# wkentaro/chainer-mask-rcnn

Measured on AMD Instinct MI355X. Metric: images/sec train step, ResNet50-C4 Mask R-CNN, COCO 800x1333, higher is better.
Workload: dtype f32 (bf16x3 split operands, f32 accumulate)

## Files before the change

chainer_mask_rcnn_amd/csrc/conv_gemm.hip:

```cpp
#include <algorithm>
#include <cstring>
#include <type_traits>

#include "common.h"

namespace {

typedef float f32x16 __attribute__((ext_vector_type(16)));

constexpr int BK = 32;
constexpr bool single_buffered(int tm, int mode)
{
    if (tm == 1) return mode == 0;
    return tm >= 2 && (mode == 0 || mode == 2);
}
constexpr int min_blocks(int tm, int mode)
{
    if (!single_buffered(tm, mode)) return 1;
    return tm == 4 ? 2 : (tm == 2 ? 3 : 6);
}
constexpr int KPAD = 4;

enum Mode { FWD = 0, DGRAD = 1, WGRAD = 2 };
constexpr bool is_fwd(int m) { return m == FWD; }
// ... 972 lines not shown
                    }
                }
                float row_scale[EG];
                if (MODE == WGRAD && p.scale) {
#pragma unroll
                    for (int q = 0; q < EG; ++q) {
                        const int e = g * EG + q;
                        const int row = m0 + wm * (32 * TM) + i * 32 + (e & 3) + 8 * (e >> 2) + 4 * lk;
                        row_scale[q] = row < p.M ? p.scale[row] : 0.f;
                    }
                }
#pragma unroll
                for (int q = 0; q < EG; ++q) {
                    float v = acc[i][j][g * EG + q];
                    if (MODE != WGRAD) {
                        if (f_bias) v += bias;
                        if (f_aff) v = v * scale + shift;
                        if (f_res) v += aux0[q];
                        if (f_acc) v += aux1[q];
                        if (f_resy) v += aux2[q] > 0.f ? aux0[q] : 0.f;
                        else if (f_resg) v += aux0[q];
                        if (f_relu) v = fmaxf(v, 0.f);
                        if (f_outm) v = aux3[q] > 0.f ? v : 0.f;
                    } else if (p.scale) {
                        v *= row_scale[q];
                    }
                    bstore1(rC, off[q], v);
                }
            }
        }
    }
}

__global__ void splitk_reduce_kernel(const float *__restrict__ ws, int splits, int64_t n,
                                     int64_t stride, float *__restrict__ out)
{
    const int64_t nv = n / 4;
    for (int64_t i = (int64_t)blockIdx.x * blockDim.x + threadIdx.x; i < nv;
         i += (int64_t)gridDim.x * blockDim.x) {
        float4 a = reinterpret_cast<const float4 *>(ws)[i];
        int s = 1;
        for (; s + 4 <= splits; s += 4) {
            const float4 v0 = reinterpret_cast<const float4 *>(ws + (s + 0) * stride)[i];
            const float4 v1 = reinterpret_cast<const float4 *>(ws + (s + 1) * stride)[i];
            const float4 v2 = reinterpret_cast<const float4 *>(ws + (s + 2) * stride)[i];
            const float4 v3 = reinterpret_cast<const float4 *>(ws + (s + 3) * stride)[i];
            a.x += v0.x; a.y += v0.y; a.z += v0.z; a.w += v0.w;
            a.x += v1.x; a.y += v1.y; a.z += v1.z; a.w += v1.w;
            a.x += v2.x; a.y += v2.y; a.z += v2.z; a.w += v2.w;
            a.x += v3.x; a.y += v3.y; a.z += v3.z; a.w += v3.w;
        }
        for (; s < splits; ++s) {
            const float4 v = reinterpret_cast<const float4 *>(ws + s * stride)[i];
            a.x += v.x; a.y += v.y; a.z += v.z; a.w += v.w;
        }
        reinterpret_cast<float4 *>(out)[i] = a;
    }
}

constexpr int64_t kSlotsBig = 512, kSlotsSmall = 1024;

int g_split_bf16 = 3;
int g_big_split_k = -1;
int g_big_split_min_slices = 16;
int g_w8_min_k = 256;
int g_w8 = 1;

int g_pw = 3;

inline bool pw_plain(const GemmParams &p)
{
    return p.R == 1 && p.S == 1 && p.stride == 1 && p.pad == 0 && p.perm_n == 0 && !p.stem && p.gp == p.sh &&
           p.gq == p.sw && p.out_mode == OUT_PLAIN;
}

inline bool k3_plain(const GemmParams &p)
{
    return p.R == 3 && p.S == 3 && p.stride == 1 && p.pad == 1 && p.perm_n == 0 && !p.stem &&
           p.out_mode == OUT_PLAIN;
}

template <int TM, int TN, int MODE>
void launch_kernel(const GemmParams &p, int64_t tiles, int splits, hipStream_t s, int batch = 1)
{
    hipEvent_t ev0, ev1;
    mrcnn::prof_take(&ev0, &ev1);
    auto go = [&](auto kernel) {
        hipExtLaunchKernelGGL(kernel, dim3((unsigned)tiles, splits, batch), dim3(256), 0, s, ev0, ev1, 0, p);
// ... 50 lines not shown
                        : (MODE == FWD ? mrcnn::PROF_CONV_FWD_128 : mrcnn::PROF_CONV_DGRAD_128) + (TM >= 2 ? 0 : 1);
    return mrcnn::ProfKernelScope(kind, flops, bytes);
}

template <int TM, int TN, int MODE>
void launch_tiles(GemmParams p, int m_lo, int m_hi, int splits, hipStream_t s)
{
    constexpr int BM = 64 * TM, BN = 64 * TN;
    p.m_lo = m_lo;
    p.M = m_hi;
    const int64_t blocks = mrcnn::ceil_div(m_hi - m_lo, BM) * mrcnn::ceil_div(p.N, BN);
    if (blocks <= 0) return;
    const auto prof = gemm_prof<TM, MODE>(p, m_hi - m_lo);
    launch_kernel<TM, TN, MODE>(p, blocks, splits, s);
}

constexpr int64_t kSplitWsBytes = 192ll << 20;

struct FixParams {
    const float *ws;
    float *C;
    const float *bias, *scale, *shift, *residual, *res_g, *res_y, *out_mask_y;
    int splits, rows, N, row0, ldc, flags;
    int perm_n, pq;
    int64_t stride;
};

__global__ void __launch_bounds__(256) splitk_epilogue_kernel(const FixParams f)
{
    const int n4 = f.N / 4;
    const int64_t i = (int64_t)blockIdx.x * blockDim.x + threadIdx.x;
    if (i >= (int64_t)f.rows * n4) return;
    const int r = (int)(i / n4), c = (int)(i - (int64_t)r * n4) * 4;
    float4 a = *reinterpret_cast<const float4 *>(f.ws + (int64_t)r * f.N + c);
    for (int s = 1; s < f.splits; ++s) {
        const float4 v = *reinterpret_cast<const float4 *>(f.ws + s * f.stride + (int64_t)r * f.N + c);
        a.x += v.x; a.y += v.y; a.z += v.z; a.w += v.w;
    }
    float v[4] = {a.x, a.y, a.z, a.w};
    int orow = f.row0 + r;
    if (f.perm_n > 0) {
        const PermRow pr = perm_row(orow, f.pq);
        if (pr.n >= f.perm_n) return;
        orow = pr.n * f.pq + pr.pos;
    }
    const int64_t off = (int64_t)orow * f.ldc + c;
#pragma unroll
    for (int k = 0; k < 4; ++k) {
        float x = v[k];
        if (f.flags & MRCNN_EPI_BIAS) x += f.bias[c + k];
        if (f.flags & MRCNN_EPI_AFFINE) x = x * f.scale[c + k] + (f.shift ? f.shift[c + k] : 0.f);
        if (f.flags & MRCNN_EPI_RESIDUAL) x += f.residual[off + k];
        if (f.flags & MRCNN_EPI_ACCUM) x += f.C[off + k];
        if (f.res_g) x += (!f.res_y || f.res_y[off + k] > 0.f) ? f.res_g[off + k] : 0.f;
        if (f.flags & MRCNN_EPI_RELU) x = fmaxf(x, 0.f);
        if (f.out_mask_y) x = f.out_mask_y[off + k] > 0.f ? x : 0.f;
        v[k] = x;
    }
    *reinterpret_cast<float4 *>(f.C + off) = make_float4(v[0], v[1], v[2], v[3]);
}

template <int MODE>
bool can_split_rows(const GemmParams &p)
{
    return p.split_ws && MODE != WGRAD && p.out_mode == OUT_PLAIN && !p.stem && p.N % 4 == 0 &&
           p.ldc == p.N;
}

int64_t fit_ws(int64_t splits, int64_t rows, int N)
{
    while (splits > 1 && rows * N * splits * 4 > kSplitWsBytes) --splits;
    return splits;
}

int64_t k_splits(int total_slices, int depth_div, int64_t target_wgs, int64_t tiles, int64_t rows, int N,
                 int64_t cap)
{
    return fit_ws(std::min<int64_t>(std::min<int64_t>(cap, total_slices / depth_div),
                                    mrcnn::ceil_div(target_wgs, tiles)),
                  rows, N);
}

template <int MODE>
void slab_sum(const GemmParams &p, int rows_lo, int splits, hipStream_t s)
{
    const int rows = p.M - rows_lo;
    FixParams f = {};
    f.ws = p.split_ws; f.C = p.C;
    f.bias = p.bias; f.scale = p.scale; f.shift = p.shift; f.residual = p.residual;
// ... 567 lines not shown
    p.scale = out_row_scale;
    p.M = Kout; p.N = R * S * C; p.Kc = (int)pixels;
    p.gp = P; p.gq = Q; p.sh = H; p.sw = W;
    p.R = R; p.S = S; p.stride = stride; p.pad = pad;
    p.lda = C; p.ldg = ldg; p.cin = C; p.ldc = R * S * C;
    const int64_t gwsz = (int64_t)Kout * R * S * C;
    const int64_t big = mrcnn::ceil_div(p.M, 128) * mrcnn::ceil_div(p.N, 128);
    const int64_t small = mrcnn::ceil_div(p.M, 64) * mrcnn::ceil_div(p.N, 64);
    const int64_t max_splits = std::min<int64_t>(64, std::max<int64_t>(1, pixels / (8 * BK)));
    const bool use_big = p.N > 64 && p.M > 64 && (big * max_splits * 2 >= kSlotsBig || g_big_min_tiles <= 1);
    const int64_t tiles = use_big ? big : small;
    if (C % (use_big ? 128 : 64) == 0 && N_ >= BK)
        p.perm_n = choose_perm(N_, P, Q, R, S, stride, pad);
    const int64_t k_extent = p.perm_n ? mrcnn::ceil_div(N_, BK) * BK * P * Q : pixels;
    const bool split_kernel = (g_split_bf16 & 1) && p.perm_n == 0;
    const int64_t slots_big = !split_kernel && single_buffered(2, WGRAD) ? 768 : kSlotsBig;
    int splits = wgrad_splits(tiles, pixels, use_big ? slots_big : kSlotsSmall);
    if (!ws) splits = 1;
    p.split_len = (int)(mrcnn::ceil_div(mrcnn::ceil_div(k_extent, splits), BK) * BK);
    splits = (int)mrcnn::ceil_div(k_extent, p.split_len);
    p.split_stride = gwsz;
    if (int rc = set_extents(p, pixels * ldg, (int64_t)N_ * H * W * C, gwsz)) return rc;
    p.C = splits > 1 ? (float *)ws : gw;
    {
        mrcnn::ProfKernelScope prof(use_big ? mrcnn::PROF_CONV_WGRAD_128 : mrcnn::PROF_CONV_WGRAD_64,
                                    2.0 * p.M * p.N * (double)pixels,
                                    4.0 * ((double)p.M * p.N + (double)pixels * (p.M + (double)C)));
        if (use_big)
            launch_kernel<2, 2, WGRAD>(p, big, splits, s);
        else
            launch_kernel<1, 1, WGRAD>(p, tiles, splits, s);
    }
    if (splits > 1) {
        const int64_t blocks = mrcnn::ceil_div(gwsz / 4, 256);
        hipLaunchKernelGGL(splitk_reduce_kernel, dim3((unsigned)blocks), dim3(256), 0, s,
                           (const float *)ws, splits, gwsz, gwsz, gw);
    }
    return mrcnn::check_launch("conv_wgrad");
}

extern "C" int mrcnn_conv2d_wgrad_ex(const mrcnn_conv_desc *d, const float *x, const float *gy,
                                     float *gw, void *ws, const float *out_row_scale,
                                     void *stream)
{
    if (int rc = check_desc(d)) return rc;
    MRCNN_REQUIRE(x && gy && gw, "conv2d_wgrad: null pointer");
    MRCNN_REQUIRE(aligned16(x) && aligned16(gy) && aligned16(gw) && (!ws || aligned16(ws)),
                  "conv2d_wgrad: pointers must be 16-byte aligned");
    return wgrad_impl(gy, d->K, x, gw, d->K, (int64_t)d->N * d->P * d->Q, d->N, d->H, d->W, d->C,
                      d->P, d->Q, d->R, d->S, d->stride, d->pad, ws, mrcnn::as_stream(stream),
                      out_row_scale);
}

extern "C" int mrcnn_conv2d_wgrad(const mrcnn_conv_desc *d, const float *x, const float *gy,
                                  float *gw, void *ws, void *stream)
{
    return mrcnn_conv2d_wgrad_ex(d, x, gy, gw, ws, nullptr, stream);
}

extern "C" int mrcnn_deconv2x2s2_fwd(const float *x, const float *w, const float *bias, float *y,
                                     int N, int H, int W, int C, int K, int epi_flags,
                                     void *stream)
{
    MRCNN_REQUIRE(x && w && y, "deconv_fwd: null pointer");
    MRCNN_REQUIRE(N > 0 && H > 0 && W > 0 && C > 0 && K > 0 && C % 4 == 0 && K % 4 == 0,
                  "deconv_fwd: bad shape");
    MRCNN_REQUIRE(aligned16(x) && aligned16(w), "deconv_fwd: x/w must be 16-byte aligned");
    MRCNN_REQUIRE((epi_flags & ~(MRCNN_EPI_BIAS | MRCNN_EPI_RELU)) == 0, "deconv_fwd: bad flags");
// ... 59 lines not shown
```

chainer_mask_rcnn_amd/csrc/conv_winograd.h:

```cpp
#pragma once

namespace {

constexpr int kXi = 36;

struct F2 { float x, y; };
__device__ __forceinline__ F2 operator+(F2 a, F2 b) { return {a.x + b.x, a.y + b.y}; }
__device__ __forceinline__ F2 operator-(F2 a, F2 b) { return {a.x - b.x, a.y - b.y}; }
__device__ __forceinline__ F2 operator*(float s, F2 a) { return {s * a.x, s * a.y}; }

template <typename T>
__device__ __forceinline__ void wino_bt(const T (&d)[6], T (&t)[6])
{
    t[0] = d[0] - 1.5f * d[1] - 2.f * d[2] + 1.5f * d[3] + d[4];
    t[1] = 2.5f * d[3] + 0.5f * d[2] - d[1] + d[4];
    t[2] = d[1] - 2.5f * d[2] + 0.5f * d[3] + d[4];
    t[3] = 2.f * (d[3] - d[1]) - d[2] + d[4];
    t[4] = 0.5f * (d[1] - d[3]) - d[2] + d[4];
    t[5] = d[1] - 1.5f * d[2] - 2.f * d[3] + 1.5f * d[4] + d[5];
}
template <typename T>
__device__ __forceinline__ void wino_at(const T (&m)[6], T (&y)[4])
{
    const T s12 = m[1] + m[2], d12 = m[1] - m[2];
// ... 79 lines not shown
#pragma unroll
        for (int i = 0; i < D; ++i) col[i] = d[i][j];
        if constexpr (GRAD_TILE) wino_g4(col, o);
        else wino_bt(col, o);
#pragma unroll
        for (int a = 0; a < 6; ++a) t[a][j] = o[a];
    }
    float *out = v + tile * C + c;
    const int64_t xi_stride = T * C;
#pragma unroll
    for (int a = 0; a < 6; ++a) {
        F2 o[6];
        if constexpr (GRAD_TILE) wino_g4(t[a], o);
        else wino_bt(t[a], o);
#pragma unroll
        for (int b = 0; b < 6; ++b)
            *reinterpret_cast<F2 *>(out + (a * 6 + b) * xi_stride) = o[b];
    }
}

struct WinoOutParams {
    const float *m;
    float *y;
    const float *scale, *shift, *mask;
    int H, W, K, TH, TW, flags;
    int64_t T;
    int *fix_count;
    int2 *fix_list;
    int fix_cap;
    float ambiguity;
};
float g_wino_ambiguity = 4e-6f;

template <bool FIXUP>
__global__ void __launch_bounds__(256) wino_output_transform_kernel(const WinoOutParams p)
{
    const int k2n = p.K >> 1;
    const int64_t idx = (int64_t)blockIdx.x * 256 + threadIdx.x;
    if (idx >= p.T * k2n) return;
    const int64_t tile = idx / k2n;
    const int k = (int)(idx - tile * k2n) * 2;
    const int tx = (int)(tile % p.TW);
    const int64_t q = tile / p.TW;
    const int ty = (int)(q % p.TH);
    const int64_t n = q / p.TH;
    const float *in = p.m + tile * p.K + k;
    const int64_t xi_stride = p.T * p.K;
    F2 m[6][6];
#pragma unroll
    for (int a = 0; a < 6; ++a)
#pragma unroll
        for (int b = 0; b < 6; ++b)
            m[a][b] = *reinterpret_cast<const F2 *>(in + (a * 6 + b) * xi_stride);
    const int y0 = 4 * ty, x0 = 4 * tx;
    const int64_t obase = (n * p.H * p.W) * p.K + k;
    F2 mk[4][4];
    if (p.mask) {
#pragma unroll
        for (int i = 0; i < 4; ++i)
#pragma unroll
            for (int j = 0; j < 4; ++j) {
                const bool ok = y0 + i < p.H && x0 + j < p.W;
                mk[i][j] = ok ? *reinterpret_cast<const F2 *>(
                                    p.mask + obase + ((int64_t)(y0 + i) * p.W + x0 + j) * p.K)
                              : F2{0.f, 0.f};
            }
    }
    F2 s[4][6];
    F2 sa[FIXUP ? 4 : 1][6];
#pragma unroll
    for (int b = 0; b < 6; ++b) {
        F2 col[6], o[4];
#pragma unroll
        for (int a = 0; a < 6; ++a) col[a] = m[a][b];
        wino_at(col, o);
#pragma unroll
        for (int i = 0; i < 4; ++i) s[i][b] = o[i];
        if constexpr (FIXUP) {
#pragma unroll
            for (int a = 0; a < 6; ++a) col[a] = F2{fabsf(col[a].x), fabsf(col[a].y)};
            wino_at_abs(col, o);
#pragma unroll
            for (int i = 0; i < 4; ++i) sa[i][b] = o[i];
        }
    }
    F2 sc = {1.f, 1.f}, sh = {0.f, 0.f};
    const bool aff = (p.flags & (MRCNN_EPI_AFFINE | MRCNN_EPI_BIAS)) != 0;
    const bool relu = (p.flags & MRCNN_EPI_RELU) != 0;
    if (aff) {
        if (p.scale) sc = *reinterpret_cast<const F2 *>(p.scale + k);
        if (p.shift) sh = *reinterpret_cast<const F2 *>(p.shift + k);
    }
#pragma unroll
    for (int i = 0; i < 4; ++i) {
        F2 o[4], ob[4];
        wino_at(s[i], o);
        if constexpr (FIXUP) wino_at_abs(sa[i], ob);
#pragma unroll
        for (int j = 0; j < 4; ++j) {
            if (y0 + i >= p.H || x0 + j >= p.W) continue;
            F2 v = o[j];
            if (aff) { v.x = v.x * sc.x + sh.x; v.y = v.y * sc.y + sh.y; }
            if constexpr (FIXUP) {
                const float bx = p.ambiguity * ob[j].x * fabsf(sc.x);
                const float by = p.ambiguity * ob[j].y * fabsf(sc.y);
                const int pix = (int)(n * p.H * p.W) + (y0 + i) * p.W + x0 + j;
                if (fabsf(v.x) < bx) {
                    const int at = atomicAdd(p.fix_count, 1);
                    if (at < p.fix_cap) p.fix_list[at] = make_int2(pix, k);
                }
                if (fabsf(v.y) < by) {
                    const int at = atomicAdd(p.fix_count, 1);
                    if (at < p.fix_cap) p.fix_list[at] = make_int2(pix, k + 1);
                }
            }
            if (relu) { v.x = fmaxf(v.x, 0.f); v.y = fmaxf(v.y, 0.f); }
            if (p.mask) {
                v.x = mk[i][j].x > 0.f ? v.x : 0.f;
                v.y = mk[i][j].y > 0.f ? v.y : 0.f;
            }
            *reinterpret_cast<F2 *>(p.y + obase + ((int64_t)(y0 + i) * p.W + x0 + j) * p.K) = v;
        }
    }
}

struct WinoFixParams {
    const float *x, *w, *scale, *shift;
    float *y;
    const int *count;
    const int2 *list;
    int cap, H, W, C, K, flags;
};
__global__ void __launch_bounds__(256) wino_fixup_kernel(const WinoFixParams p)
{
    const int lane = threadIdx.x & 63;
    const int wave = (int)((blockIdx.x * 256 + threadIdx.x) >> 6), nwaves = (int)(gridDim.x * 4);
    const int n_items = min(*p.count, p.cap);
    for (int it = wave; it < n_items; it += nwaves) {
        const int2 e = p.list[it];
        const int pix = e.x, k = e.y;
        const int n = pix / (p.H * p.W), rem = pix - n * (p.H * p.W);
        const int yy = rem / p.W, xx = rem - yy * p.W;
        float acc = 0.f;
        for (int r = 0; r < 3; ++r) {
            const int iy = yy + r - 1;
            if ((unsigned)iy >= (unsigned)p.H) continue;
            for (int s = 0; s < 3; ++s) {
                const int ix = xx + s - 1;
                if ((unsigned)ix >= (unsigned)p.W) continue;
                const float *xp = p.x + ((int64_t)(n * p.H + iy) * p.W + ix) * p.C;
                const float *wp = p.w + ((int64_t)k * 9 + r * 3 + s) * p.C;
                for (int c = lane * 4; c < p.C; c += 256) {
                    const float4 a = *reinterpret_cast<const float4 *>(xp + c);
                    const float4 b = *reinterpret_cast<const float4 *>(wp + c);
                    acc += (a.x * b.x + a.y * b.y) + (a.z * b.z + a.w * b.w);
                }
            }
        }
#pragma unroll
        for (int off = 32; off > 0; off >>= 1) acc += __shfl_down(acc, off, 64);
        if (lane == 0) {
            float v = acc;
            if (p.flags & (MRCNN_EPI_AFFINE | MRCNN_EPI_BIAS))
                v = v * (p.scale ? p.scale[k] : 1.f) + (p.shift ? p.shift[k] : 0.f);
            if (p.flags & MRCNN_EPI_RELU) v = fmaxf(v, 0.f);
            p.y[(int64_t)pix * p.K + k] = v;
        }
    }
}

template <bool TRANSPOSED>
__global__ void __launch_bounds__(256) wino_filter_transform_kernel(
    const float *__restrict__ w, float *__restrict__ u, int K, int C,
    const float *__restrict__ row_scale)
{
    __shared__ float tile[32][33];
    const int k0 = blockIdx.y * 32, c0 = blockIdx.x * 32;
    const int tx = threadIdx.x & 31, ty = threadIdx.x >> 5;
    double f[4][9];
#pragma unroll
    for (int j = 0; j < 4; ++j) {
        const int k = k0 + ty + 8 * j, c = c0 + tx;
        const bool ok = k < K && c < C;
        const double rsc = (TRANSPOSED && row_scale && ok) ? (double)row_scale[k] : 1.0;
#pragma unroll
        for (int rs = 0; rs < 9; ++rs) {
            const int src = TRANSPOSED ? 8 - rs : rs;
            f[j][rs] = ok ? (double)w[((int64_t)k * 9 + src) * C + c] * rsc : 0.0;
        }
    }
    for (int a = 0; a < 6; ++a)
        for (int b = 0; b < 6; ++b) {
            float val[4];
#pragma unroll
            for (int j = 0; j < 4; ++j) {
                double acc = 0.0;
#pragma unroll
                for (int r = 0; r < 3; ++r) {
                    const double row = kFilterG[b][0] * f[j][r * 3] + kFilterG[b][1] * f[j][r * 3 + 1] +
                                       kFilterG[b][2] * f[j][r * 3 + 2];
                    acc += kFilterG[a][r] * row;
                }
                val[j] = (float)acc;
            }
            float *dst = u + (int64_t)(a * 6 + b) * K * C;
            if constexpr (!TRANSPOSED) {
#pragma unroll
                for (int j = 0; j < 4; ++j) {
                    const int k = k0 + ty + 8 * j, c = c0 + tx;
                    if (k < K && c < C) dst[(int64_t)k * C + c] = val[j];
                }
            } else {
                __syncthreads();
#pragma unroll
                for (int j = 0; j < 4; ++j) tile[ty + 8 * j][tx] = val[j];
                __syncthreads();
#pragma unroll
                for (int j = 0; j < 4; ++j) {
                    const int c = c0 + ty + 8 * j, k = k0 + tx;
                    if (c < C && k < K) dst[(int64_t)c * K + k] = tile[tx][ty + 8 * j];
                }
            }
        }
}

__global__ void __launch_bounds__(256) wino_wgrad_finish_kernel(
    const float *__restrict__ slabs, int splits, int64_t split_stride, float *__restrict__ gw,
    const float *__restrict__ row_scale, int K, int C)
{
    const int64_t idx = (int64_t)blockIdx.x * 256 + threadIdx.x;
    if (idx >= (int64_t)K * C) return;
    const int k = (int)(idx / C), c = (int)(idx - (int64_t)k * C);
    const int64_t kc = (int64_t)K * C;
    float du[kXi];
#pragma unroll
    for (int xi = 0; xi < kXi; ++xi) du[xi] = slabs[xi * kc + idx];
    for (int s = 1; s < splits; ++s) {
        const float *sl = slabs + s * split_stride;
#pragma unroll
        for (int xi = 0; xi < kXi; ++xi) du[xi] += sl[xi * kc + idx];
    }
    const double rsc = row_scale ? (double)row_scale[k] : 1.0;
    double t[3][6];
#pragma unroll
    for (int r = 0; r < 3; ++r)
#pragma unroll
        for (int b = 0; b < 6; ++b) {
            double acc = 0.0;
#pragma unroll
            for (int a = 0; a < 6; ++a) acc += kWgradAT[r][a] * (double)du[a * 6 + b];
            t[r][b] = acc;
        }
#pragma unroll
    for (int r = 0; r < 3; ++r)
#pragma unroll
        for (int s = 0; s < 3; ++s) {
// ... 68 lines not shown
        launch_kernel<1, 1, FWD>(q, mrcnn::ceil_div(p.N, 64), 1, s, kXi);
    } else if (big) {
        launch_kernel<2, 2, FWD>(p, tiles, 1, s, kXi);
    } else {
        launch_kernel<1, 1, FWD>(p, tiles, 1, s, kXi);
    }
    return mrcnn::check_launch("wino_batched_gemm");
}

}

extern "C" int64_t mrcnn_conv3x3_wino_v_bytes(const mrcnn_conv_desc *d)
{
    return d ? 4 * wino_plane_floats(d, d->C) : 0;
}

extern "C" int64_t mrcnn_conv3x3_wino_workspace_bytes(const mrcnn_conv_desc *d)
{
    if (!d) return 0;
    const int64_t ch = std::max(d->C, d->K);
    return 4 * ((1 + kWinoMaxSplits) * wino_u_floats(d) + 2 * wino_plane_floats(d, (int)ch));
}

extern "C" int64_t mrcnn_conv3x3_wino_u_bytes(const mrcnn_conv_desc *d)
{
    return d ? 4 * wino_u_floats(d) : 0;
}

extern "C" int mrcnn_conv3x3_wino_filter(const mrcnn_conv_desc *d, const float *w, float *u,
                                         void *stream)
{
    if (int rc = wino_check(d, "conv3x3_wino_filter")) return rc;
    MRCNN_REQUIRE(w && u, "conv3x3_wino_filter: null pointer");
    hipLaunchKernelGGL((wino_filter_transform_kernel<false>),
                       dim3((d->C + 31) / 32, (d->K + 31) / 32), dim3(256), 0,
                       mrcnn::as_stream(stream), w, u, d->K, d->C, (const float *)nullptr);
    return mrcnn::check_launch("conv3x3_wino_filter");
}

extern "C" int mrcnn_conv3x3_wino_fwd(const mrcnn_conv_desc *d, const float *x, const float *w,
                                      const float *u_pre, const float *scale, const float *shift,
                                      float *y, int epi_flags, float *v, void *ws, void *stream)
{
    if (int rc = wino_check(d, "conv3x3_wino_fwd")) return rc;
    MRCNN_REQUIRE(x && (w || u_pre) && y && ws, "conv3x3_wino_fwd: null pointer");
    MRCNN_REQUIRE((epi_flags & ~(MRCNN_EPI_AFFINE | MRCNN_EPI_BIAS | MRCNN_EPI_RELU |
                                 MRCNN_EPI_EXACT_SIGNS)) == 0,
                  "conv3x3_wino_fwd: only AFFINE or BIAS, RELU and EXACT_SIGNS");
    MRCNN_REQUIRE(!(epi_flags & MRCNN_EPI_EXACT_SIGNS) || w,
                  "conv3x3_wino_fwd: EXACT_SIGNS needs the filter itself");
    MRCNN_REQUIRE(!(epi_flags & MRCNN_EPI_AFFINE) || scale, "conv3x3_wino_fwd: affine flag without scale");
    MRCNN_REQUIRE(!(epi_flags & MRCNN_EPI_BIAS) || (shift && !scale && !(epi_flags & MRCNN_EPI_AFFINE)),
                  "conv3x3_wino_fwd: the bias flag takes the bias in `shift` and excludes AFFINE");
    hipStream_t s = mrcnn::as_stream(stream);
    const WinoGeom g = wino_geom(d);
    float *u_ws = (float *)ws;
    float *m = u_ws + wino_u_floats(d);
    float *vbuf = v ? v : m + wino_plane_floats(d, d->K);
    const float *u = u_pre;
    if (!u) {
        hipLaunchKernelGGL((wino_filter_transform_kernel<false>),
                           dim3((d->C + 31) / 32, (d->K + 31) / 32), dim3(256), 0, s, w, u_ws, d->K,
                           d->C, (const float *)nullptr);
        u = u_ws;
    }
    wino_launch_data_transform<false>(x, vbuf, g, d->C, s);
    if (int rc = wino_batched_gemm(vbuf, u, m, g.T, d->K, d->C, s)) return rc;
    WinoOutParams o = {};
    o.m = m; o.y = y; o.scale = scale; o.shift = shift;
    o.H = d->H; o.W = d->W; o.K = d->K; o.TH = g.TH; o.TW = g.TW;
    o.flags = epi_flags & ~MRCNN_EPI_EXACT_SIGNS; o.T = g.T;
    const bool fixup = (epi_flags & MRCNN_EPI_EXACT_SIGNS) != 0;
    if (fixup) {
        float *fix = (float *)ws + wino_u_floats(d) + 2 * wino_plane_floats(d, std::max(d->C, d->K));
        o.fix_count = (int *)fix;
        o.fix_list = (int2 *)(fix + 4);
        o.fix_cap = (int)std::min<int64_t>(1 << 20, (8 * wino_u_floats(d) - 4) / 2);
        o.ambiguity = g_wino_ambiguity;
        MRCNN_HIP_TRY(hipMemsetAsync(o.fix_count, 0, 16, s));
    }
    {
        mrcnn::ProfScope prof(mrcnn::PROF_WINO_TRANSFORM, 0.,
                              4.0 * d->K * (36.0 * g.T + (double)d->N * d->H * d->W), s);
        const dim3 grid((unsigned)mrcnn::ceil_div(g.T * (d->K / 2), 256));
        if (fixup) hipLaunchKernelGGL(wino_output_transform_kernel<true>, grid, dim3(256), 0, s, o);
        else hipLaunchKernelGGL(wino_output_transform_kernel<false>, grid, dim3(256), 0, s, o);
    }
    if (fixup) {
        WinoFixParams f = {};
        f.x = x; f.w = w; f.scale = scale; f.shift = shift; f.y = y;
        f.count = o.fix_count; f.list = o.fix_list; f.cap = o.fix_cap;
        f.H = d->H; f.W = d->W; f.C = d->C; f.K = d->K; f.flags = o.flags;
        hipLaunchKernelGGL(wino_fixup_kernel, dim3(1024), dim3(256), 0, s, f);
    }
    return mrcnn::check_launch("conv3x3_wino_fwd");
}

extern "C" int mrcnn_conv3x3_wino_dgrad(const mrcnn_conv_desc *d, const float *gy, const float *w,
                                        const float *w_row_scale, float *gx,
                                        const float *out_scale, const float *out_mask_y, void *ws,
                                        void *stream)
{
    if (int rc = wino_check(d, "conv3x3_wino_dgrad")) return rc;
    MRCNN_REQUIRE(gy && w && gx && ws, "conv3x3_wino_dgrad: null pointer");
    hipStream_t s = mrcnn::as_stream(stream);
    const WinoGeom g = wino_geom(d);
    const int64_t ch = std::max(d->C, d->K);
    float *u = (float *)ws;
    float *gt = u + (1 + kWinoMaxSplits) * wino_u_floats(d);
    float *m = gt + wino_plane_floats(d, (int)ch);
    hipLaunchKernelGGL((wino_filter_transform_kernel<true>),
                       dim3((d->C + 31) / 32, (d->K + 31) / 32), dim3(256), 0, s, w, u, d->K, d->C,
                       w_row_scale);
    wino_launch_data_transform<false>(gy, gt, g, d->K, s);
    if (int rc = wino_batched_gemm(gt, u, m, g.T, d->C, d->K, s)) return rc;
    WinoOutParams o = {};
    o.m = m; o.y = gx; o.scale = out_scale; o.mask = out_mask_y;
    o.H = d->H; o.W = d->W; o.K = d->C; o.TH = g.TH; o.TW = g.TW;
    o.flags = out_scale ? MRCNN_EPI_AFFINE : 0; o.T = g.T;
    {
        mrcnn::ProfScope prof(mrcnn::PROF_WINO_TRANSFORM, 0.,
                              4.0 * d->C * (36.0 * g.T + (out_mask_y ? 2.0 : 1.0) * d->N * d->H * d->W), s);
        hipLaunchKernelGGL(wino_output_transform_kernel<false>,
                           dim3((unsigned)mrcnn::ceil_div(g.T * (d->C / 2), 256)), dim3(256), 0, s, o);
    }
    return mrcnn::check_launch("conv3x3_wino_dgrad");
}

extern "C" int mrcnn_conv3x3_wino_wgrad(const mrcnn_conv_desc *d, const float *x, const float *v,
                                        const float *gy, float *gw, const float *out_row_scale,
                                        void *ws, void *stream)
{
    if (int rc = wino_check(d, "conv3x3_wino_wgrad")) return rc;
    MRCNN_REQUIRE((x != nullptr) != (v != nullptr), "conv3x3_wino_wgrad: exactly one of x / v");
    MRCNN_REQUIRE(gy && gw && ws, "conv3x3_wino_wgrad: null pointer");
    hipStream_t s = mrcnn::as_stream(stream);
    const WinoGeom g = wino_geom(d);
    float *slabs = (float *)ws + wino_u_floats(d);
    float *gt = (float *)ws + (1 + kWinoMaxSplits) * wino_u_floats(d);
    if (!v) {
        float *vx = gt + wino_plane_floats(d, std::max(d->C, d->K));
        wino_launch_data_transform<false>(x, vx, g, d->C, s);
        v = vx;
    }
    wino_launch_data_transform<true>(gy, gt, g, d->K, s);
    GemmParams p = {};
    p.A = gt; p.B = v;
    p.M = d->K; p.N = d->C; p.Kc = (int)g.T;
    p.gp = p.gq = p.sh = p.sw = 1;
    p.R = p.S = 1; p.stride = 1; p.pad = 0;
    p.lda = d->C; p.ldg = d->K; p.cin = d->C; p.ldc = d->C;
    const int64_t kc = (int64_t)d->K * d->C;
    const bool big = p.M > 64 && p.N > 64;
    const int64_t tiles = big ? mrcnn::ceil_div(p.M, 128) * mrcnn::ceil_div(p.N, 128)
                              : mrcnn::ceil_div(p.M, 64) * mrcnn::ceil_div(p.N, 64);
    const int64_t slots = big ? (single_buffered(2, WGRAD) ? 768 : kSlotsBig) : kSlotsSmall;
    int splits = std::min(kWinoMaxSplits, wgrad_splits(tiles * kXi, g.T, slots));
// ... 30 lines not shown
```

chainer_mask_rcnn_amd/csrc/elementwise.hip:

```cpp
#include <algorithm>

#include "common.h"

namespace {

constexpr int kColsumSplits = 128;

__global__ void affine_fwd_kernel(const float *__restrict__ x, const float *__restrict__ W,
                                  const float *__restrict__ b, float *__restrict__ y,
                                  int64_t total, int C)
{
    for (int64_t i = (int64_t)blockIdx.x * blockDim.x + threadIdx.x; i < total;
         i += (int64_t)gridDim.x * blockDim.x) {
        const int c = (int)(i % C);
        y[i] = W[c] * x[i] + b[c];
    }
}

template <bool VEC>
__global__ void epilogue_bwd_kernel(const float *__restrict__ gy, const float *__restrict__ y,
                                    const float *__restrict__ scale, float *__restrict__ g,
                                    int64_t total, int C)
{
    if (VEC) {
// ... 67 lines not shown
        for (; s < splits; s += 4) a0 += partial[(int64_t)s * C + c];
    }
    red[g][cx] = (a0 + a1) + (a2 + a3);
    __syncthreads();
    if (g == 0 && c < C) out[c] = (red[0][cx] + red[1][cx]) + (red[2][cx] + red[3][cx]);
}

template <typename V>
__device__ __forceinline__ V vmax(V a, V b);
template <> __device__ __forceinline__ float vmax(float a, float b) { return fmaxf(a, b); }
template <> __device__ __forceinline__ float4 vmax(float4 a, float4 b)
{
    return make_float4(fmaxf(a.x, b.x), fmaxf(a.y, b.y), fmaxf(a.z, b.z), fmaxf(a.w, b.w));
}
template <typename V> __device__ __forceinline__ V vneginf();
template <> __device__ __forceinline__ float vneginf() { return -INFINITY; }
template <> __device__ __forceinline__ float4 vneginf()
{
    return make_float4(-INFINITY, -INFINITY, -INFINITY, -INFINITY);
}

template <typename V>
__global__ void maxpool_kernel(const V *__restrict__ x, V *__restrict__ y, int N, int H, int W,
                               int CV, int P, int Q)
{
    const int64_t total = (int64_t)N * P * Q * CV;
    for (int64_t i = (int64_t)blockIdx.x * blockDim.x + threadIdx.x; i < total;
         i += (int64_t)gridDim.x * blockDim.x) {
        const int c = (int)(i % CV);
        int64_t t = i / CV;
        const int q = (int)(t % Q); t /= Q;
        const int p = (int)(t % P);
        const int n = (int)(t / P);
        V m = vneginf<V>();
#pragma unroll
        for (int r = 0; r < 3; ++r) {
            const int iy = 2 * p - 1 + r;
            if (iy < 0 || iy >= H) continue;
#pragma unroll
            for (int s = 0; s < 3; ++s) {
                const int ix = 2 * q - 1 + s;
                if (ix < 0 || ix >= W) continue;
                m = vmax(m, x[(((int64_t)n * H + iy) * W + ix) * CV + c]);
            }
        }
        y[i] = m;
    }
}

template <bool VEC>
__global__ void avgpool_fwd_kernel(const float *__restrict__ x, float *__restrict__ y, int R,
                                   int HW, int C)
{
    const int w = VEC ? 4 : 1;
    const int cv = C / w;
    const int64_t i = (int64_t)blockIdx.x * blockDim.x + threadIdx.x;
    if (i >= (int64_t)R * cv) return;
    const int r = (int)(i / cv), c = (int)(i % cv);
    const float inv = 1.f / (float)HW;
    if (VEC) {
        const float4 *p = reinterpret_cast<const float4 *>(x) + (int64_t)r * HW * cv + c;
        float4 a = make_float4(0.f, 0.f, 0.f, 0.f);
        for (int k = 0; k < HW; ++k) {
            const float4 v = p[(int64_t)k * cv];
            a.x += v.x; a.y += v.y; a.z += v.z; a.w += v.w;
        }
        reinterpret_cast<float4 *>(y)[i] = make_float4(a.x * inv, a.y * inv, a.z * inv, a.w * inv);
    } else {
        const float *p = x + (int64_t)r * HW * C + c;
        float a = 0.f;
        for (int k = 0; k < HW; ++k) a += p[(int64_t)k * C];
        y[i] = a * inv;
    }
}

template <bool VEC>
__global__ void avgpool_bwd_kernel(const float *__restrict__ gy, float *__restrict__ gx, int R,
// ... 232 lines not shown
namespace {
__global__ void __launch_bounds__(256)
sparse3x3_gather_kernel(const float4 *__restrict__ x, const float4 *__restrict__ g,
                        const int32_t *__restrict__ rows, int H, int W, int C4, int K4,
                        float4 *__restrict__ patches, float4 *__restrict__ g_rows)
{
    const int i = blockIdx.x, t = blockIdx.y;
    const int p = rows[i];
    if (t == 9) {
        const float4 *src = g + (int64_t)p * K4;
        float4 *dst = g_rows + (int64_t)i * K4;
        for (int c = threadIdx.x; c < K4; c += blockDim.x) dst[c] = src[c];
        return;
    }
    const int px = p % W, py = (p / W) % H, n = p / (W * H);
    const int yy = py + t / 3 - 1, xx = px + t % 3 - 1;
    const bool in = (unsigned)yy < (unsigned)H && (unsigned)xx < (unsigned)W;
    const float4 *src = x + (((int64_t)n * H + yy) * W + xx) * C4;
    float4 *dst = patches + ((int64_t)i * 9 + t) * C4;
    const float4 zero = make_float4(0.f, 0.f, 0.f, 0.f);
    for (int c = threadIdx.x; c < C4; c += blockDim.x) dst[c] = in ? src[c] : zero;
}

__global__ void __launch_bounds__(256)
sparse3x3_scatter_kernel(const float4 *__restrict__ gp, const int32_t *__restrict__ lookup, int H,
                         int W, int C4, float4 *__restrict__ gx)
{
    const int q = blockIdx.x;
    const int qx = q % W, qy = (q / W) % H, n = q / (W * H);
    int src[9];
#pragma unroll
    for (int t = 0; t < 9; ++t) {
        const int yy = qy - (t / 3 - 1), xx = qx - (t % 3 - 1);
        src[t] = ((unsigned)yy < (unsigned)H && (unsigned)xx < (unsigned)W)
                     ? lookup[((int64_t)n * H + yy) * W + xx] : -1;
    }
    for (int c = threadIdx.x; c < C4; c += blockDim.x) {
        float4 acc = make_float4(0.f, 0.f, 0.f, 0.f);
#pragma unroll
        for (int t = 0; t < 9; ++t) {
            if (src[t] < 0) continue;
            const float4 v = gp[((int64_t)src[t] * 9 + t) * C4 + c];
            acc.x += v.x; acc.y += v.y; acc.z += v.z; acc.w += v.w;
        }
        gx[(int64_t)q * C4 + c] = acc;
    }
}
}

extern "C" int mrcnn_sparse3x3_gather(const float *x, const float *g, const int32_t *rows,
                                      int n_rows, int N, int H, int W, int C, int K,
                                      float *patches, float *g_rows, void *stream)
{
    MRCNN_REQUIRE(n_rows >= 0 && N > 0 && H > 0 && W > 0 && C > 0 && K > 0 && C % 4 == 0 &&
                      K % 4 == 0, "sparse3x3_gather: bad shape");
    if (n_rows == 0) return 0;
    MRCNN_REQUIRE(x && g && rows && patches && g_rows, "sparse3x3_gather: null pointer");
    mrcnn::ProfScope prof(mrcnn::PROF_ELEMENTWISE, 0.,
                          8.0 * (double)n_rows * (9.0 * C + K), mrcnn::as_stream(stream));
    hipLaunchKernelGGL(sparse3x3_gather_kernel, dim3(n_rows, 10), dim3(256), 0,
                       mrcnn::as_stream(stream), (const float4 *)x, (const float4 *)g, rows, H, W,
                       C / 4, K / 4, (float4 *)patches, (float4 *)g_rows);
    return mrcnn::check_launch("sparse3x3_gather");
}

extern "C" int mrcnn_sparse3x3_scatter(const float *g_patches, const int32_t *lookup, int N, int H,
                                       int W, int C, float *gx, void *stream)
{
    MRCNN_REQUIRE(N > 0 && H > 0 && W > 0 && C > 0 && C % 4 == 0, "sparse3x3_scatter: bad shape");
    MRCNN_REQUIRE((int64_t)N * H * W < (int64_t)INT32_MAX, "sparse3x3_scatter: map too large");
    MRCNN_REQUIRE(g_patches && lookup && gx, "sparse3x3_scatter: null pointer");
    hipLaunchKernelGGL(sparse3x3_scatter_kernel, dim3(N * H * W), dim3(256), 0,
                       mrcnn::as_stream(stream), (const float4 *)g_patches, lookup, H, W, C / 4,
                       (float4 *)gx);
    return mrcnn::check_launch("sparse3x3_scatter");
}

extern "C" int mrcnn_sgd_momentum_wd_ex(float *p, float *g, float *v, int64_t n, float lr,
// ... 25 lines not shown
```

Before: 90.92.

## Batch loads ahead of use in reduce, epilogue, winograd, pooling and scatter kernels

Several memory-bound helper kernels are restructured so that their global loads are issued unconditionally up front, using clamped or dummy addresses, before any data-dependent branching. This raises memory-level parallelism in the split-K reduce and epilogue, the winograd output and filter transforms, max pooling and the sparse 3x3 scatter. The winograd filter transform gets a new thread mapping with an LDS transpose tile, the masked output transform becomes a template specialisation, and the reduce launch uses smaller blocks for small outputs. The cost is some extra loads and more register pressure.

```diff
diff --git a/chainer_mask_rcnn_amd/csrc/conv_gemm.hip b/chainer_mask_rcnn_amd/csrc/conv_gemm.hip
--- a/chainer_mask_rcnn_amd/csrc/conv_gemm.hip
+++ b/chainer_mask_rcnn_amd/csrc/conv_gemm.hip
@@ -1028,28 +1028,40 @@
     }
 }
 
+
+constexpr int kSlabGroup = 8;
+
+__device__ __forceinline__ void add4(float4 &a, const float4 &v)
+{
+    a.x += v.x; a.y += v.y; a.z += v.z; a.w += v.w;
+}
+
+template <bool WHOLE>
+__device__ __forceinline__ void add_slab_group(float4 &a, const float *base, int64_t stride, int s0,
+                                               int splits)
+{
+    float4 v[kSlabGroup];
+#pragma unroll
+    for (int j = 0; j < kSlabGroup; ++j) {
+        const int s = WHOLE ? s0 + j : min(s0 + j, splits - 1);
+        v[j] = *reinterpret_cast<const float4 *>(base + s * stride);
+    }
+#pragma unroll
+    for (int j = 0; j < kSlabGroup; ++j)
+        if (WHOLE || s0 + j < splits) add4(a, v[j]);
+}
+
 __global__ void splitk_reduce_kernel(const float *__restrict__ ws, int splits, int64_t n,
                                      int64_t stride, float *__restrict__ out)
 {
     const int64_t nv = n / 4;
     for (int64_t i = (int64_t)blockIdx.x * blockDim.x + threadIdx.x; i < nv;
          i += (int64_t)gridDim.x * blockDim.x) {
-        float4 a = reinterpret_cast<const float4 *>(ws)[i];
+        const float *base = ws + 4 * i;
+        float4 a = *reinterpret_cast<const float4 *>(base);
         int s = 1;
-        for (; s + 4 <= splits; s += 4) {
-            const float4 v0 = reinterpret_cast<const float4 *>(ws + (s + 0) * stride)[i];
-            const float4 v1 = reinterpret_cast<const float4 *>(ws + (s + 1) * stride)[i];
-            const float4 v2 = reinterpret_cast<const float4 *>(ws + (s + 2) * stride)[i];
-            const float4 v3 = reinterpret_cast<const float4 *>(ws + (s + 3) * stride)[i];
-            a.x += v0.x; a.y += v0.y; a.z += v0.z; a.w += v0.w;
-            a.x += v1.x; a.y += v1.y; a.z += v1.z; a.w += v1.w;
-            a.x += v2.x; a.y += v2.y; a.z += v2.z; a.w += v2.w;
-            a.x += v3.x; a.y += v3.y; a.z += v3.z; a.w += v3.w;
-        }
-        for (; s < splits; ++s) {
-            const float4 v = reinterpret_cast<const float4 *>(ws + s * stride)[i];
-            a.x += v.x; a.y += v.y; a.z += v.z; a.w += v.w;
-        }
+        for (; s + kSlabGroup <= splits; s += kSlabGroup) add_slab_group<true>(a, base, stride, s, splits);
+        if (s < splits) add_slab_group<false>(a, base, stride, s, splits);
         reinterpret_cast<float4 *>(out)[i] = a;
     }
 }
@@ -1166,12 +1178,6 @@
     const int64_t i = (int64_t)blockIdx.x * blockDim.x + threadIdx.x;
     if (i >= (int64_t)f.rows * n4) return;
     const int r = (int)(i / n4), c = (int)(i - (int64_t)r * n4) * 4;
-    float4 a = *reinterpret_cast<const float4 *>(f.ws + (int64_t)r * f.N + c);
-    for (int s = 1; s < f.splits; ++s) {
-        const float4 v = *reinterpret_cast<const float4 *>(f.ws + s * f.stride + (int64_t)r * f.N + c);
-        a.x += v.x; a.y += v.y; a.z += v.z; a.w += v.w;
-    }
-    float v[4] = {a.x, a.y, a.z, a.w};
     int orow = f.row0 + r;
     if (f.perm_n > 0) {
         const PermRow pr = perm_row(orow, f.pq);
@@ -1179,16 +1185,51 @@
         orow = pr.n * f.pq + pr.pos;
     }
     const int64_t off = (int64_t)orow * f.ldc + c;
+    const float *slab0 = f.ws + (int64_t)r * f.N + c;
+    const bool f_bias = (f.flags & MRCNN_EPI_BIAS) != 0, f_aff = (f.flags & MRCNN_EPI_AFFINE) != 0;
+    const bool f_shift = f_aff && f.shift != nullptr;
+    const bool f_res = (f.flags & MRCNN_EPI_RESIDUAL) != 0, f_acc = (f.flags & MRCNN_EPI_ACCUM) != 0;
+    const bool f_resg = f.res_g != nullptr, f_resy = f_resg && f.res_y != nullptr;
+    const bool f_relu = (f.flags & MRCNN_EPI_RELU) != 0, f_outm = f.out_mask_y != nullptr;
+    auto ld4 = [](const float *q) { return *reinterpret_cast<const float4 *>(q); };
+    const float4 bias4 = ld4(f_bias ? f.bias + c : slab0);
+    const float4 scale4 = ld4(f_aff ? f.scale + c : slab0);
+    const float4 shift4 = ld4(f_shift ? f.shift + c : slab0);
+    const float4 res4 = ld4(f_res ? f.residual + off : slab0);
+    const float4 acc4 = ld4(f_acc ? f.C + off : slab0);
+    const float4 resg4 = ld4(f_resg ? f.res_g + off : slab0);
+    const float4 resy4 = ld4(f_resy ? f.res_y + off : slab0);
+    const float4 outm4 = ld4(f_outm ? f.out_mask_y + off : slab0);
+    float4 a = make_float4(0.f, 0.f, 0.f, 0.f);
+    {
+        float4 sv[kSlabGroup];
+#pragma unroll
+        for (int j = 0; j < kSlabGroup; ++j) sv[j] = ld4(slab0 + min(j, f.splits - 1) * f.stride);
+        a = sv[0];
+#pragma unroll
+        for (int j = 1; j < kSlabGroup; ++j)
+            if (j < f.splits) add4(a, sv[j]);
+    }
+    for (int s = kSlabGroup; s < f.splits; s += kSlabGroup) add_slab_group<false>(a, slab0, f.stride, s, f.splits);
+    float v[4] = {a.x, a.y, a.z, a.w};
+    const float b[4] = {bias4.x, bias4.y, bias4.z, bias4.w};
+    const float sc[4] = {scale4.x, scale4.y, scale4.z, scale4.w};
+    const float sh[4] = {shift4.x, shift4.y, shift4.z, shift4.w};
+    const float r0[4] = {res4.x, res4.y, res4.z, res4.w};
+    const float r1[4] = {acc4.x, acc4.y, acc4.z, acc4.w};
+    const float rg[4] = {resg4.x, resg4.y, resg4.z, resg4.w};
+    const float ry[4] = {resy4.x, resy4.y, resy4.z, resy4.w};
+    const float om[4] = {outm4.x, outm4.y, outm4.z, outm4.w};
 #pragma unroll
     for (int k = 0; k < 4; ++k) {
         float x = v[k];
-        if (f.flags & MRCNN_EPI_BIAS) x += f.bias[c + k];
-        if (f.flags & MRCNN_EPI_AFFINE) x = x * f.scale[c + k] + (f.shift ? f.shift[c + k] : 0.f);
-        if (f.flags & MRCNN_EPI_RESIDUAL) x += f.residual[off + k];
-        if (f.flags & MRCNN_EPI_ACCUM) x += f.C[off + k];
-        if (f.res_g) x += (!f.res_y || f.res_y[off + k] > 0.f) ? f.res_g[off + k] : 0.f;
-        if (f.flags & MRCNN_EPI_RELU) x = fmaxf(x, 0.f);
-        if (f.out_mask_y) x = f.out_mask_y[off + k] > 0.f ? x : 0.f;
+        if (f_bias) x += b[k];
+        if (f_aff) x = x * sc[k] + (f_shift ? sh[k] : 0.f);
+        if (f_res) x += r0[k];
+        if (f_acc) x += r1[k];
+        if (f_resg) x += (!f_resy || ry[k] > 0.f) ? rg[k] : 0.f;
+        if (f_relu) x = fmaxf(x, 0.f);
+        if (f_outm) x = om[k] > 0.f ? x : 0.f;
         v[k] = x;
     }
     *reinterpret_cast<float4 *>(f.C + off) = make_float4(v[0], v[1], v[2], v[3]);
@@ -1822,8 +1863,9 @@
             launch_kernel<1, 1, WGRAD>(p, tiles, splits, s);
     }
     if (splits > 1) {
-        const int64_t blocks = mrcnn::ceil_div(gwsz / 4, 256);
-        hipLaunchKernelGGL(splitk_reduce_kernel, dim3((unsigned)blocks), dim3(256), 0, s,
+        const int threads = gwsz / 4 < (64 << 10) ? 64 : 256;
+        const int64_t blocks = mrcnn::ceil_div(gwsz / 4, threads);
+        hipLaunchKernelGGL(splitk_reduce_kernel, dim3((unsigned)blocks), dim3(threads), 0, s,
                            (const float *)ws, splits, gwsz, gwsz, gw);
     }
     return mrcnn::check_launch("conv_wgrad");
diff --git a/chainer_mask_rcnn_amd/csrc/conv_winograd.h b/chainer_mask_rcnn_amd/csrc/conv_winograd.h
--- a/chainer_mask_rcnn_amd/csrc/conv_winograd.h
+++ b/chainer_mask_rcnn_amd/csrc/conv_winograd.h
@@ -135,7 +135,7 @@
 };
 float g_wino_ambiguity = 4e-6f;
 
-template <bool FIXUP>
+template <bool FIXUP, bool MASKED>
 __global__ void __launch_bounds__(256) wino_output_transform_kernel(const WinoOutParams p)
 {
     const int k2n = p.K >> 1;
@@ -157,18 +157,21 @@
             m[a][b] = *reinterpret_cast<const F2 *>(in + (a * 6 + b) * xi_stride);
     const int y0 = 4 * ty, x0 = 4 * tx;
     const int64_t obase = (n * p.H * p.W) * p.K + k;
-    F2 mk[4][4];
-    if (p.mask) {
+    F2 mk[MASKED ? 4 : 1][4];
+    if constexpr (MASKED) {
 #pragma unroll
         for (int i = 0; i < 4; ++i)
 #pragma unroll
             for (int j = 0; j < 4; ++j) {
-                const bool ok = y0 + i < p.H && x0 + j < p.W;
-                mk[i][j] = ok ? *reinterpret_cast<const F2 *>(
-                                    p.mask + obase + ((int64_t)(y0 + i) * p.W + x0 + j) * p.K)
-                              : F2{0.f, 0.f};
+                const int yy = min(y0 + i, p.H - 1), xx = min(x0 + j, p.W - 1);
+                mk[i][j] = *reinterpret_cast<const F2 *>(p.mask + obase + ((int64_t)yy * p.W + xx) * p.K);
             }
     }
+    const bool aff = (p.flags & (MRCNN_EPI_AFFINE | MRCNN_EPI_BIAS)) != 0;
+    const bool relu = (p.flags & MRCNN_EPI_RELU) != 0;
+    const bool has_sc = aff && p.scale != nullptr, has_sh = aff && p.shift != nullptr;
+    const F2 sc_ld = *reinterpret_cast<const F2 *>(has_sc ? p.scale + k : in);
+    const F2 sh_ld = *reinterpret_cast<const F2 *>(has_sh ? p.shift + k : in);
     F2 s[4][6];
     F2 sa[FIXUP ? 4 : 1][6];
 #pragma unroll
@@ -187,13 +190,7 @@
             for (int i = 0; i < 4; ++i) sa[i][b] = o[i];
         }
     }
-    F2 sc = {1.f, 1.f}, sh = {0.f, 0.f};
-    const bool aff = (p.flags & (MRCNN_EPI_AFFINE | MRCNN_EPI_BIAS)) != 0;
-    const bool relu = (p.flags & MRCNN_EPI_RELU) != 0;
-    if (aff) {
-        if (p.scale) sc = *reinterpret_cast<const F2 *>(p.scale + k);
-        if (p.shift) sh = *reinterpret_cast<const F2 *>(p.shift + k);
-    }
+    const F2 sc = has_sc ? sc_ld : F2{1.f, 1.f}, sh = has_sh ? sh_ld : F2{0.f, 0.f};
 #pragma unroll
     for (int i = 0; i < 4; ++i) {
         F2 o[4], ob[4];
@@ -218,7 +215,7 @@
                 }
             }
             if (relu) { v.x = fmaxf(v.x, 0.f); v.y = fmaxf(v.y, 0.f); }
-            if (p.mask) {
+            if constexpr (MASKED) {
                 v.x = mk[i][j].x > 0.f ? v.x : 0.f;
                 v.y = mk[i][j].y > 0.f ? v.y : 0.f;
             }
@@ -272,59 +269,74 @@
     }
 }
 
+constexpr int kFtK = 32, kFtC = 8, kFtLd = kFtK + 8;
 template <bool TRANSPOSED>
 __global__ void __launch_bounds__(256) wino_filter_transform_kernel(
     const float *__restrict__ w, float *__restrict__ u, int K, int C,
     const float *__restrict__ row_scale)
 {
-    __shared__ float tile[32][33];
-    const int k0 = blockIdx.y * 32, c0 = blockIdx.x * 32;
-    const int tx = threadIdx.x & 31, ty = threadIdx.x >> 5;
-    double f[4][9];
-#pragma unroll
-    for (int j = 0; j < 4; ++j) {
-        const int k = k0 + ty + 8 * j, c = c0 + tx;
-        const bool ok = k < K && c < C;
-        const double rsc = (TRANSPOSED && row_scale && ok) ? (double)row_scale[k] : 1.0;
-#pragma unroll
-        for (int rs = 0; rs < 9; ++rs) {
-            const int src = TRANSPOSED ? 8 - rs : rs;
-            f[j][rs] = ok ? (double)w[((int64_t)k * 9 + src) * C + c] * rsc : 0.0;
-        }
-    }
+    __shared__ float tile[TRANSPOSED ? kXi * kFtC * kFtLd : 1];
+    int k, c;
+    if constexpr (TRANSPOSED) {
+        k = blockIdx.y * kFtK + (threadIdx.x >> 3);
+        c = blockIdx.x * kFtC + (threadIdx.x & 7);
+    } else {
+        const int64_t idx = (int64_t)blockIdx.x * 256 + threadIdx.x;
+        k = (int)(idx / C);
+        c = (int)(idx - (int64_t)k * C);
+    }
+    const bool ok = k < K && c < C;
+    const int kk = min(k, K - 1), cc = min(c, C - 1);
+    const bool scaled = TRANSPOSED && row_scale != nullptr;
+    const float rs = *(scaled ? row_scale + kk : w);
+    float tap[9];
+#pragma unroll
+    for (int rs9 = 0; rs9 < 9; ++rs9) {
+        const int src = TRANSPOSED ? 8 - rs9 : rs9;
+        tap[rs9] = w[((int64_t)kk * 9 + src) * C + cc];
+    }
+    const double rsc = (scaled && ok) ? (double)rs : 1.0;
+    double f[9];
+#pragma unroll
+    for (int rs9 = 0; rs9 < 9; ++rs9) f[rs9] = ok ? (double)tap[rs9] * rsc : 0.0;
+    double row[6][3];
+#pragma unroll
+    for (int b = 0; b < 6; ++b)
+#pragma unroll
+        for (int r = 0; r < 3; ++r)
+            row[b][r] = kFilterG[b][0] * f[r * 3] + kFilterG[b][1] * f[r * 3 + 1] +
+                        kFilterG[b][2] * f[r * 3 + 2];
+    const int64_t kc = (int64_t)K * C;
+#pragma unroll
     for (int a = 0; a < 6; ++a)
+#pragma unroll
         for (int b = 0; b < 6; ++b) {
-            float val[4];
-#pragma unroll
-            for (int j = 0; j < 4; ++j) {
-                double acc = 0.0;
-#pragma unroll
-                for (int r = 0; r < 3; ++r) {
-                    const double row = kFilterG[b][0] * f[j][r * 3] + kFilterG[b][1] * f[j][r * 3 + 1] +
-                                       kFilterG[b][2] * f[j][r * 3 + 2];
-                    acc += kFilterG[a][r] * row;
-                }
-                val[j] = (float)acc;
-            }
-            float *dst = u + (int64_t)(a * 6 + b) * K * C;
-            if constexpr (!TRANSPOSED) {
-#pragma unroll
-                for (int j = 0; j < 4; ++j) {
-                    const int k = k0 + ty + 8 * j, c = c0 + tx;
-                    if (k < K && c < C) dst[(int64_t)k * C + c] = val[j];
-                }
-            } else {
-                __syncthreads();
-#pragma unroll
-                for (int j = 0; j < 4; ++j) tile[ty + 8 * j][tx] = val[j];
-                __syncthreads();
-#pragma unroll
-                for (int j = 0; j < 4; ++j) {
-                    const int c = c0 + ty + 8 * j, k = k0 + tx;
-                    if (c < C && k < K) dst[(int64_t)c * K + k] = tile[tx][ty + 8 * j];
-                }
-            }
-        }
+            double acc = 0.0;
+#pragma unroll
+            for (int r = 0; r < 3; ++r) acc += kFilterG[a][r] * row[b][r];
+            const float val = (float)acc;
+            if constexpr (TRANSPOSED) tile[((a * 6 + b) * kFtC + (threadIdx.x & 7)) * kFtLd + (threadIdx.x >> 3)] = val;
+            else if (ok) u[(a * 6 + b) * kc + (int64_t)k * C + c] = val;
+        }
+    if constexpr (TRANSPOSED) {
+        __syncthreads();
+        const int tk = threadIdx.x & 31, tc = threadIdx.x >> 5;
+        const int ko = blockIdx.y * kFtK + tk, co = blockIdx.x * kFtC + tc;
+        if (ko < K && co < C) {
+#pragma unroll
+            for (int xi = 0; xi < kXi; ++xi) u[xi * kc + (int64_t)co * K + ko] = tile[(xi * kFtC + tc) * kFtLd + tk];
+        }
+    }
+}
+
+template <bool TRANSPOSED>
+void wino_launch_filter_transform(const float *w, float *u, int K, int C, const float *row_scale,
+                                  hipStream_t s)
+{
+    const dim3 grid = TRANSPOSED ? dim3((C + kFtC - 1) / kFtC, (K + kFtK - 1) / kFtK)
+                                 : dim3((unsigned)mrcnn::ceil_div((int64_t)K * C, 256));
+    hipLaunchKernelGGL((wino_filter_transform_kernel<TRANSPOSED>), grid, dim3(256), 0, s, w, u, K, C,
+                       row_scale);
 }
 
 __global__ void __launch_bounds__(256) wino_wgrad_finish_kernel(
@@ -459,9 +471,7 @@
 {
     if (int rc = wino_check(d, "conv3x3_wino_filter")) return rc;
     MRCNN_REQUIRE(w && u, "conv3x3_wino_filter: null pointer");
-    hipLaunchKernelGGL((wino_filter_transform_kernel<false>),
-                       dim3((d->C + 31) / 32, (d->K + 31) / 32), dim3(256), 0,
-                       mrcnn::as_stream(stream), w, u, d->K, d->C, (const float *)nullptr);
+    wino_launch_filter_transform<false>(w, u, d->K, d->C, nullptr, mrcnn::as_stream(stream));
     return mrcnn::check_launch("conv3x3_wino_filter");
 }
 
@@ -486,9 +496,7 @@
     float *vbuf = v ? v : m + wino_plane_floats(d, d->K);
     const float *u = u_pre;
     if (!u) {
-        hipLaunchKernelGGL((wino_filter_transform_kernel<false>),
-                           dim3((d->C + 31) / 32, (d->K + 31) / 32), dim3(256), 0, s, w, u_ws, d->K,
-                           d->C, (const float *)nullptr);
+        wino_launch_filter_transform<false>(w, u_ws, d->K, d->C, nullptr, s);
         u = u_ws;
     }
     wino_launch_data_transform<false>(x, vbuf, g, d->C, s);
@@ -510,8 +518,8 @@
         mrcnn::ProfScope prof(mrcnn::PROF_WINO_TRANSFORM, 0.,
                               4.0 * d->K * (36.0 * g.T + (double)d->N * d->H * d->W), s);
         const dim3 grid((unsigned)mrcnn::ceil_div(g.T * (d->K / 2), 256));
-        if (fixup) hipLaunchKernelGGL(wino_output_transform_kernel<true>, grid, dim3(256), 0, s, o);
-        else hipLaunchKernelGGL(wino_output_transform_kernel<false>, grid, dim3(256), 0, s, o);
+        if (fixup) hipLaunchKernelGGL((wino_output_transform_kernel<true, false>), grid, dim3(256), 0, s, o);
+        else hipLaunchKernelGGL((wino_output_transform_kernel<false, false>), grid, dim3(256), 0, s, o);
     }
     if (fixup) {
         WinoFixParams f = {};
@@ -536,9 +544,7 @@
     float *u = (float *)ws;
     float *gt = u + (1 + kWinoMaxSplits) * wino_u_floats(d);
     float *m = gt + wino_plane_floats(d, (int)ch);
-    hipLaunchKernelGGL((wino_filter_transform_kernel<true>),
-                       dim3((d->C + 31) / 32, (d->K + 31) / 32), dim3(256), 0, s, w, u, d->K, d->C,
-                       w_row_scale);
+    wino_launch_filter_transform<true>(w, u, d->K, d->C, w_row_scale, s);
     wino_launch_data_transform<false>(gy, gt, g, d->K, s);
     if (int rc = wino_batched_gemm(gt, u, m, g.T, d->C, d->K, s)) return rc;
     WinoOutParams o = {};
@@ -548,8 +554,9 @@
     {
         mrcnn::ProfScope prof(mrcnn::PROF_WINO_TRANSFORM, 0.,
                               4.0 * d->C * (36.0 * g.T + (out_mask_y ? 2.0 : 1.0) * d->N * d->H * d->W), s);
-        hipLaunchKernelGGL(wino_output_transform_kernel<false>,
-                           dim3((unsigned)mrcnn::ceil_div(g.T * (d->C / 2), 256)), dim3(256), 0, s, o);
+        const dim3 grid((unsigned)mrcnn::ceil_div(g.T * (d->C / 2), 256));
+        if (out_mask_y) hipLaunchKernelGGL((wino_output_transform_kernel<false, true>), grid, dim3(256), 0, s, o);
+        else hipLaunchKernelGGL((wino_output_transform_kernel<false, false>), grid, dim3(256), 0, s, o);
     }
     return mrcnn::check_launch("conv3x3_wino_dgrad");
 }
diff --git a/chainer_mask_rcnn_amd/csrc/elementwise.hip b/chainer_mask_rcnn_amd/csrc/elementwise.hip
--- a/chainer_mask_rcnn_amd/csrc/elementwise.hip
+++ b/chainer_mask_rcnn_amd/csrc/elementwise.hip
@@ -123,17 +123,18 @@
         const int q = (int)(t % Q); t /= Q;
         const int p = (int)(t % P);
         const int n = (int)(t / P);
+        V v[9];
+#pragma unroll
+        for (int t = 0; t < 9; ++t) {
+            const int iy = min(max(2 * p - 1 + t / 3, 0), H - 1), ix = min(max(2 * q - 1 + t % 3, 0), W - 1);
+            v[t] = x[(((int64_t)n * H + iy) * W + ix) * CV + c];
+        }
         V m = vneginf<V>();
 #pragma unroll
-        for (int r = 0; r < 3; ++r) {
-            const int iy = 2 * p - 1 + r;
-            if (iy < 0 || iy >= H) continue;
-#pragma unroll
-            for (int s = 0; s < 3; ++s) {
-                const int ix = 2 * q - 1 + s;
-                if (ix < 0 || ix >= W) continue;
-                m = vmax(m, x[(((int64_t)n * H + iy) * W + ix) * CV + c]);
-            }
+        for (int t = 0; t < 9; ++t) {
+            const int iy = 2 * p - 1 + t / 3, ix = 2 * q - 1 + t % 3;
+            const bool ok = iy >= 0 && iy < H && ix >= 0 && ix < W;
+            m = ok ? vmax(m, v[t]) : m;
         }
         y[i] = m;
     }
@@ -432,18 +433,26 @@
 #pragma unroll
     for (int t = 0; t < 9; ++t) {
         const int yy = qy - (t / 3 - 1), xx = qx - (t % 3 - 1);
-        src[t] = ((unsigned)yy < (unsigned)H && (unsigned)xx < (unsigned)W)
-                     ? lookup[((int64_t)n * H + yy) * W + xx] : -1;
+        src[t] = lookup[((int64_t)n * H + min(max(yy, 0), H - 1)) * W + min(max(xx, 0), W - 1)];
+    }
+#pragma unroll
+    for (int t = 0; t < 9; ++t) {
+        const int yy = qy - (t / 3 - 1), xx = qx - (t % 3 - 1);
+        if ((unsigned)yy >= (unsigned)H || (unsigned)xx >= (unsigned)W) src[t] = -1;
     }
     for (int c = threadIdx.x; c < C4; c += blockDim.x) {
+        float4 *out = gx + (int64_t)q * C4 + c;
+        float4 v[9];
+#pragma unroll
+        for (int t = 0; t < 9; ++t)
+            v[t] = *(src[t] >= 0 ? gp + ((int64_t)src[t] * 9 + t) * C4 + c : out);
         float4 acc = make_float4(0.f, 0.f, 0.f, 0.f);
 #pragma unroll
         for (int t = 0; t < 9; ++t) {
             if (src[t] < 0) continue;
-            const float4 v = gp[((int64_t)src[t] * 9 + t) * C4 + c];
-            acc.x += v.x; acc.y += v.y; acc.z += v.z; acc.w += v.w;
-        }
-        gx[(int64_t)q * C4 + c] = acc;
+            acc.x += v[t].x; acc.y += v[t].y; acc.z += v[t].z; acc.w += v[t].w;
+        }
+        *out = acc;
     }
 }
 }
```

Measured after the change: 92.06 (median of 6 runs). +1.3%, better.
